# dedis/kyber

Hardware: AMD Instinct MI355X
Metric: scalar-muls/s + pairings/s per node; MSM sec at 2^20 points (higher is better)
Workload: dtype int32 limbs (radix 2^25.5), int64 accumulate; 1 GPU; Ed25519 batched fixed-base + var-base scalar-mul, 2^20 scalars per GPU (BASELINE.json configs[1]); elements_per_gpu=1048576

## Files before the change

kyber_amd/csrc/ed25519.hip:

```cpp
#ifndef KYB_TU_WAVES
#define KYB_TU_WAVES 2
#endif
#include "context.h"
#include "ed25519_dev.cuh"
#include "ed25519_launch.h"
#include "msm.cuh"
#include "ed25519_h2c.cuh"
#include <stdlib.h>
#include <string.h>

#include <algorithm>
#include <atomic>
#include <chrono>
#include <thread>
#include <vector>

namespace kyb {


template <int G = 2>
__global__ void ed25519_build_base_table_kernel(int32_t* __restrict__ tab, const uint32_t* __restrict__ point,
                                                uint32_t* __restrict__ ok, int rows = ED_TAB_POS * ED_TAB_ENT) {
    const int t = blockIdx.x * blockDim.x + threadIdx.x;
    if (t >= rows) return;
    ge_p3 B;
    if (point) {
        uint32_t pw[8];
        load_words8(pw, point);
        const bool good = ge_p3_fromwords(B, pw);
        if (t == 0) *ok = good ? 1u : 0u;
    } else {
        B.X = fe_bx(); B.Y = fe_by(); fe_1(B.Z); B.T = fe_bt();
    }
    ed_comb_row<G>(tab + (size_t)t * ED_TAB_STRIDE, t, B);
}

__global__ __launch_bounds__(64, KYB_TU_WAVES) void ed25519_encode_kernel(size_t n, const int32_t* __restrict__ proj,
                                                            const uint8_t* __restrict__ status,
                                                            uint32_t* __restrict__ out) {
    ed_encode_chunk(n, proj, (size_t)blockIdx.x * blockDim.x + threadIdx.x, [&](size_t i, uint32_t (&w)[8]) {
        if (status && status[i]) {
#pragma unroll
            for (int k = 0; k < 8; k++) w[k] = 0;
        }
        store_words8(out + i * 8, w);
    });
}


template <int G>
__global__ __launch_bounds__(256, 3) void ed25519_mul_base_kernel(
    size_t n, const uint32_t* __restrict__ scalars, uint32_t* __restrict__ out,
    const int32_t* __restrict__ tab, uint32_t flags, int32_t* __restrict__ proj) {
    const bool full = (flags & KYB_F_VARTIME) != 0;
    for (size_t idx = (size_t)blockIdx.x * blockDim.x + threadIdx.x; idx < n;
         idx += (size_t)gridDim.x * blockDim.x) {
        uint32_t a[8];
        load_words8(a, scalars + idx * 8);
        int8_t e[65];
        recode16(e, a, full);
        ge_p3 h;
        ge_p3_0(h);
        ge_precomp t;
        ge_p1p1 r;
        const int npos = full ? EdComb<G>::POS : EdComb<G>::POS_CT;
#pragma unroll 1
        for (int k = 0; k < npos; k++) {
            int d = 0;
#pragma unroll
            for (int i = G - 1; i >= 0; i--)
                if (G * k + i <= 64) d = 16 * d + (int)e[G * k + i];
            if (full && __ballot(d != 0) == 0) continue;
            select_precomp_tab<EdComb<G>::ENT>(t, tab, k, d);
            ge_madd(r, h, t);
            ge_p1p1_to_p3(h, r);
        }
        if (proj) {
            store_proj(proj, idx, h);
            continue;
        }
        uint32_t w[8];
        ge_p3_towords(w, h);
        store_words8(out + idx * 8, w);
    }
}

KYB_DEV void select_precomp_uniform(ge_precomp& t, const int32_t* __restrict__ tab, int i, int b) {
    const bool neg = b < 0;
    const int babs = neg ? -b : b;
    const int pos = i >> 1, mult = (i & 1) ? 16 : 1;
    fe_1(t.ypx);
    fe_1(t.ymx);
    fe_0(t.xy2d);
#pragma unroll 1
    for (int m = 1; m <= 8; m++) {
        const int4* e = reinterpret_cast<const int4*>(tab + (size_t)(pos * ED_TAB_ENT + (m * mult - 1)) * ED_TAB_STRIDE);
        int32_t w[32];
#pragma unroll
        for (int q = 0; q < 8; q++) {
            const int4 x = e[q];
            w[4 * q] = x.x;
            w[4 * q + 1] = x.y;
            w[4 * q + 2] = x.z;
            w[4 * q + 3] = x.w;
        }
        const int32_t keep = -(int32_t)(babs == m);
#pragma unroll
        for (int l = 0; l < 10; l++) {
            t.ypx.v[l] ^= (t.ypx.v[l] ^ w[l]) & keep;
            t.ymx.v[l] ^= (t.ymx.v[l] ^ w[10 + l]) & keep;
            t.xy2d.v[l] ^= (t.xy2d.v[l] ^ w[20 + l]) & keep;
        }
    }
    ge_precomp_cneg(t, neg);
}
__global__ __launch_bounds__(256, 3) void ed25519_mul_base_uniform_kernel(
    size_t n, const uint32_t* __restrict__ scalars, uint32_t* __restrict__ out,
    const int32_t* __restrict__ tab, int32_t* __restrict__ proj) {
    for (size_t idx = (size_t)blockIdx.x * blockDim.x + threadIdx.x; idx < n;
         idx += (size_t)gridDim.x * blockDim.x) {
        uint32_t a[8];
        load_words8(a, scalars + idx * 8);
        int8_t e[65];
        recode16(e, a, false);
        ge_p3 h;
        ge_p3_0(h);
        ge_precomp t;
        ge_p1p1 r;
#pragma unroll 1
        for (int i = 0; i < 64; i++) {
            select_precomp_uniform(t, tab, i, (int)e[i]);
            ge_madd(r, h, t);
            ge_p1p1_to_p3(h, r);
        }
        if (proj) {
            store_proj(proj, idx, h);
            continue;
        }
        uint32_t w[8];
        ge_p3_towords(w, h);
        store_words8(out + idx * 8, w);
    }
}


template <bool GTAB, bool UNI = false>
__global__ __launch_bounds__(128, 3) void ed25519_mul_kernel(
    size_t n, const uint32_t* __restrict__ scalars, const uint32_t* __restrict__ points,
    size_t points_stride, uint32_t* __restrict__ out, uint8_t* __restrict__ status,
    uint32_t flags, int32_t* __restrict__ proj, int4* __restrict__ gtab) {
    const size_t idx = (size_t)blockIdx.x * blockDim.x + threadIdx.x;
    if (idx >= n) return;
    const bool full = !UNI && (flags & KYB_F_VARTIME) != 0;
    uint32_t pw[8], a[8];
    load_words8(pw, points + idx * points_stride);
    load_words8(a, scalars + idx * 8);
    ge_p3 A;
    const bool ok = ge_p3_fromwords(A, pw);
    int8_t e[65];
    recode16(e, a, full);
    ge_p3 h;
    const int vt_top = full ? wave_top_digit(a) : 63;
    if constexpr (GTAB) {
        TabGlobal tab{gtab + idx * 80};
        ge_scalarmult_w4<UNI>(h, e, A, full, tab, vt_top);
    } else {
        TabScratch tab;
        ge_scalarmult_w4<UNI>(h, e, A, full, tab, vt_top);
    }
    if (proj) {
        store_proj(proj, idx, h);
        if (status) status[idx] = ok ? KYB_ST_OK : KYB_ST_BAD_POINT;
        return;
    }
    uint32_t w[8];
    ge_p3_towords(w, h);
    if (!ok) {
#pragma unroll
        for (int i = 0; i < 8; i++) w[i] = 0;
    }
    store_words8(out + idx * 8, w);
    if (status) status[idx] = ok ? KYB_ST_OK : KYB_ST_BAD_POINT;
}

int ed25519_build_tables(DeviceCtx* ctx) {
    KYB_HIP_CHECK(hipMalloc(&ctx->ed_base_tab, ED_TAB_WORDS * sizeof(int32_t)));
    hipLaunchKernelGGL(ed25519_build_base_table_kernel<2>, dim3((ED_TAB_POS * ED_TAB_ENT + 63) / 64), dim3(64), 0,
                       nullptr, ctx->ed_base_tab, (const uint32_t*)nullptr, (uint32_t*)nullptr, ED_TAB_POS * ED_TAB_ENT);
    KYB_HIP_CHECK(hipGetLastError());
    const auto t0 = std::chrono::steady_clock::now();
    KYB_HIP_CHECK(hipMalloc(&ctx->ed_wide_tab, ED_WIDE_WORDS * sizeof(int32_t)));
    hipLaunchKernelGGL(ed25519_build_base_table_kernel<ED_COMB_G>, dim3((EdWide::ROWS + 63) / 64), dim3(64), 0, nullptr,
                       ctx->ed_wide_tab, (const uint32_t*)nullptr, (uint32_t*)nullptr, EdWide::ROWS);
    KYB_HIP_CHECK(hipGetLastError());
    KYB_HIP_CHECK(hipStreamSynchronize(nullptr));
    ctx->ed_wide_build_us = std::chrono::duration_cast<std::chrono::microseconds>(std::chrono::steady_clock::now() - t0).count();
    return KYB_OK;
}
void ed25519_free_tables(DeviceCtx* ctx) {
    if (ctx->ed_base_tab) hipFree(ctx->ed_base_tab);
    if (ctx->ed_wide_tab) hipFree(ctx->ed_wide_tab);
    ctx->ed_base_tab = ctx->ed_wide_tab = nullptr;
}

constexpr size_t ENC_DEFER_MIN = 4096;


static int launch_mul_base(DeviceCtx* ctx, size_t n, const void* d_scalars, void* d_out, uint32_t flags,
                           hipStream_t st, const int32_t* tab = nullptr) {
    const bool wide = !tab && !(flags & KYB_F_UNIFORM);
    if (!tab) tab = wide ? ctx->ed_wide_tab : ctx->ed_base_tab;
    if (n == 0) return KYB_OK;
    const int block = 256;
    size_t want = (n + block - 1) / block;
    size_t cap = (size_t)ctx->num_cu * 8;
    int grid = (int)(want < cap ? want : cap);
    EdSlab w{};
    std::lock_guard<std::recursive_mutex> enq_lock(ctx->enq_mu);
    if (n >= ENC_DEFER_MIN)
        if (int rc = ed_slab(ctx, st, ED_SLAB_MUL_BASE, n, &w)) return rc;
    if (flags & KYB_F_UNIFORM) {
        hipLaunchKernelGGL(ed25519_mul_base_uniform_kernel, dim3(grid), dim3(block), 0, st, n,
                           (const uint32_t*)d_scalars, (uint32_t*)d_out, tab, w.proj);
    } else {
        const auto kernel = wide ? ed25519_mul_base_kernel<ED_COMB_G> : ed25519_mul_base_kernel<2>;
        hipLaunchKernelGGL(kernel, dim3(grid), dim3(block), 0, st, n, (const uint32_t*)d_scalars, (uint32_t*)d_out, tab,
                           flags, w.proj);
    }
    if (w.proj)
        hipLaunchKernelGGL(ed25519_encode_kernel, ed_encode_grid(n), dim3(ED_ENC_BLOCK), 0, st, n, w.proj,
                           (const uint8_t*)nullptr, (uint32_t*)d_out);
    KYB_HIP_CHECK(hipGetLastError());
    return KYB_OK;
}
static int launch_mul(size_t n, const void* d_scalars, const void* d_points, size_t stride, void* d_out,
                      void* d_status, uint32_t flags, hipStream_t st) {
    if (n == 0) return KYB_OK;
    const int block = 128;
    size_t grid = (n + block - 1) / block;
    EdSlab w{};
    uint8_t* stat = (uint8_t*)d_status;
    DeviceCtx* ctx;
    int rc = get_ctx(&ctx);
    if (rc) return rc;
    std::lock_guard<std::recursive_mutex> enq_lock(ctx->enq_mu);
    const bool defer = n >= ENC_DEFER_MIN, uni = (flags & KYB_F_UNIFORM) != 0;
    const auto kernel = defer ? (uni ? ed25519_mul_kernel<true, true> : ed25519_mul_kernel<true, false>)
                              : (uni ? ed25519_mul_kernel<false, true> : ed25519_mul_kernel<false, false>);
    if (defer) {
        if ((rc = ed_slab(ctx, st, ed_slab_mul(stat == nullptr), n, &w))) return rc;
        if (!stat) stat = w.status;
    }
    hipLaunchKernelGGL(kernel, dim3((unsigned)grid), dim3(block), 0, st, n, (const uint32_t*)d_scalars,
                       (const uint32_t*)d_points, stride, (uint32_t*)d_out, stat, flags, w.proj, w.gtab);
    if (w.proj)
        hipLaunchKernelGGL(ed25519_encode_kernel, ed_encode_grid(n), dim3(ED_ENC_BLOCK), 0, st, n, w.proj,
                           (const uint8_t*)stat, (uint32_t*)d_out);
    KYB_HIP_CHECK(hipGetLastError());
    return KYB_OK;
}

}

using namespace kyb;

static bool ed_mul_flags_bad(uint32_t flags) {
    return (flags & ~(KYB_F_VARTIME | KYB_F_UNIFORM)) || (flags & (KYB_F_VARTIME | KYB_F_UNIFORM)) == (KYB_F_VARTIME | KYB_F_UNIFORM);
}

extern "C" {

int kyb_ed25519_mul_base_dev(size_t n, const void* d_scalars, void* d_out, uint32_t flags, void* stream) {
    if ((n && (!d_scalars || !d_out)) || ed_mul_flags_bad(flags)) {
        set_error("kyb_ed25519_mul_base_dev: bad argument");
        return KYB_E_ARG;
    }
    DeviceCtx* ctx;
    int rc = get_ctx(&ctx);
    if (rc) return rc;
    return launch_mul_base(ctx, n, d_scalars, d_out, flags, (hipStream_t)stream);
}

int kyb_ed25519_mul_dev(size_t n, const void* d_scalars, const void* d_points, void* d_out, void* d_status,
                        uint32_t flags, void* stream) {
    if ((n && (!d_scalars || !d_points || !d_out)) || ed_mul_flags_bad(flags)) {
        set_error("kyb_ed25519_mul_dev: bad argument");
        return KYB_E_ARG;
    }
    DeviceCtx* ctx;
    int rc = get_ctx(&ctx);
    if (rc) return rc;
    return launch_mul(n, d_scalars, d_points, 8, d_out, d_status, flags, (hipStream_t)stream);
}

static int mul_host(size_t n, const uint8_t* scalars, const uint8_t* points, size_t stride, uint8_t* out,
                    uint8_t* status, uint32_t flags);

int kyb_ed25519_mul_base(size_t n, const uint8_t* scalars, uint8_t* out, uint32_t flags) {
    if ((n && (!scalars || !out)) || ed_mul_flags_bad(flags)) {
        set_error("kyb_ed25519_mul_base: bad argument");
        return KYB_E_ARG;
    }
    if (n == 0) return KYB_OK;
    if (md_active(n))
        return md_run(n, [&](int, size_t lo, size_t hi) { return kyb_ed25519_mul_base(hi - lo, scalars + 32 * lo, out + 32 * lo, flags); });
    return mul_host(n, scalars, nullptr, 0, out, nullptr, flags);
}

constexpr size_t PIPE_CHUNK_MAX = PIN_SLOT_ELEMS;
constexpr int PIPE_SLOTS = DeviceCtx::NPIN, PIPE_STREAMS = 3;
static size_t pipe_chunk(const DeviceCtx* ctx) {
    if (const char* e = getenv("KYB_PIPE_CHUNK")) {
        const size_t v = (size_t)strtoull(e, nullptr, 10) & ~size_t(63);
        if (v >= 4096) return std::min(PIPE_CHUNK_MAX, v);
    }
    (void)ctx;
    return size_t(1) << 17;
}
static int pipe_nstreams() {
    if (const char* e = getenv("KYB_PIPE_STREAMS")) {
        const int v = atoi(e);
        if (v >= 1 && v <= PIPE_STREAMS) return v;
    }
    return 2;
}
constexpr size_t SAME_BASE_TABLE_MIN = 16384;

static int pipe_streams(DeviceCtx::StagePool* pool) {
    for (int i = 0; i < PIPE_STREAMS; i++)
        if (!pool->pipe[i]) KYB_HIP_CHECK(hipStreamCreateWithFlags(&pool->pipe[i], hipStreamNonBlocking));
    return KYB_OK;
}

static int mul_host(size_t n, const uint8_t* scalars, const uint8_t* points, size_t stride, uint8_t* out,
                    uint8_t* status, uint32_t flags) {
    DeviceCtx* ctx;
    int rc = get_ctx(&ctx);
    if (rc) return rc;
    bool fixed = points == nullptr;
    const size_t npts = fixed ? 0 : (stride ? n : 1);
    StageScope sc_(ctx);
    StageBuf d_s, d_p, d_o, d_st, d_tab;
    if ((rc = d_s.alloc(n * 32))) return rc;
    if ((rc = d_p.alloc(npts * 32))) return rc;
    if ((rc = d_o.alloc(n * 32))) return rc;
    if ((rc = d_st.alloc(n))) return rc;
    const int32_t* tab = nullptr;
    if (!fixed && !stride && (n >= SAME_BASE_TABLE_MIN || (flags & KYB_F_UNIFORM))) {
        if ((rc = d_tab.alloc(ED_TAB_WORDS * sizeof(int32_t) + 256))) return rc;
        uint32_t* d_ok = (uint32_t*)((uint8_t*)d_tab.p + ED_TAB_WORDS * sizeof(int32_t));
        KYB_HIP_CHECK(hipMemcpy(d_p.p, points, 32, hipMemcpyHostToDevice));
        hipLaunchKernelGGL(ed25519_build_base_table_kernel<2>, dim3((ED_TAB_POS * ED_TAB_ENT + 63) / 64), dim3(64), 0, sc_.stream(),
                           (int32_t*)d_tab.p, (const uint32_t*)d_p.p, d_ok, ED_TAB_POS * ED_TAB_ENT);
        uint32_t ok = 0;
        KYB_HIP_CHECK(hipMemcpy(&ok, d_ok, 4, hipMemcpyDeviceToHost));
        if (!ok) {
            memset(out, 0, n * 32);
            if (status) memset(status, KYB_ST_BAD_POINT, n);
            return KYB_OK;
        }
        if (status) memset(status, 0, n);
        tab = (const int32_t*)d_tab.p;
        fixed = true;
    }
    auto launch = [&](size_t off, size_t cnt, hipStream_t st) -> int {
        uint8_t* s = (uint8_t*)d_s.p + off * 32;
        uint8_t* o = (uint8_t*)d_o.p + off * 32;
        if (fixed) return launch_mul_base(ctx, cnt, s, o, flags, st, tab);
        const uint8_t* p = (const uint8_t*)d_p.p + (stride ? off * 32 : 0);
        return launch_mul(cnt, s, p, stride, o, (uint8_t*)d_st.p + off, flags, st);
    };
    const size_t PIPE_CHUNK = pipe_chunk(ctx);
    if (n < 2 * PIPE_CHUNK) {
        KYB_HIP_CHECK(hipMemcpy(d_s.p, scalars, n * 32, hipMemcpyHostToDevice));
        if (npts) KYB_HIP_CHECK(hipMemcpy(d_p.p, points, npts * 32, hipMemcpyHostToDevice));
        if ((rc = launch(0, n, nullptr))) return rc;
        if ((rc = d_o.download(out, n * 32))) return rc;
        if (status && !fixed) rc = d_st.download(status, n);
        return rc;
    }
    DeviceCtx::StagePool* pool = sc_.pool;
    if ((rc = pipe_streams(pool))) return rc;
    const int nstreams = pipe_nstreams();
    const bool per_point = !fixed && stride;
    const bool want_status = status && !fixed;
    if ((rc = ctx_pin_slots(pool))) return rc;
    const size_t nchunks = (n + PIPE_CHUNK - 1) / PIPE_CHUNK;
    std::vector<hipEvent_t> ev_out(nchunks);
    for (size_t i = 0; i < nchunks; i++) KYB_HIP_CHECK(hipEventCreateWithFlags(&ev_out[i], hipEventDisableTiming));
    auto enqueue = [&](size_t i) -> int {
        const size_t off = i * PIPE_CHUNK, cnt = std::min(PIPE_CHUNK, n - off);
        uint8_t* pin = (uint8_t*)pool->pin_in[i % PIPE_SLOTS];
        uint8_t* pout = (uint8_t*)pool->pin_out[i % PIPE_SLOTS];
        hipStream_t s_k = pool->pipe[i % nstreams];
        par_memcpy(pin, scalars + off * 32, cnt * 32);
        if (per_point) par_memcpy(pin + PIPE_CHUNK_MAX * 32, points + off * 32, cnt * 32);
        int r;
        if (fixed) {
            r = launch_mul_base(ctx, cnt, pin, pout, flags, s_k, tab);
        } else {
            const uint8_t* p = per_point ? pin + PIPE_CHUNK_MAX * 32 : (const uint8_t*)d_p.p;
            r = launch_mul(cnt, pin, p, stride, pout, (uint8_t*)d_st.p + off, flags, s_k);
        }
        if (r) return r;
        if (want_status)
            KYB_HIP_CHECK(hipMemcpyAsync(pout + PIPE_CHUNK_MAX * 32, (uint8_t*)d_st.p + off, cnt, hipMemcpyDeviceToHost, s_k));
        KYB_HIP_CHECK(hipEventRecord(ev_out[i], s_k));
        return KYB_OK;
    };
    auto drain = [&](size_t i) -> int {
        const size_t off = i * PIPE_CHUNK, cnt = std::min(PIPE_CHUNK, n - off);
        KYB_HIP_CHECK(hipEventSynchronize(ev_out[i]));
        const uint8_t* pout = (const uint8_t*)pool->pin_out[i % PIPE_SLOTS];
        par_memcpy(out + off * 32, pout, cnt * 32);
        if (want_status) memcpy(status + off, pout + PIPE_CHUNK_MAX * 32, cnt);
        return KYB_OK;
    };
    if (!fixed && !stride) KYB_HIP_CHECK(hipMemcpy(d_p.p, points, 32, hipMemcpyHostToDevice));
    std::atomic<size_t> enqueued{0}, drained{0};
    std::atomic<int> drain_rc{KYB_OK};
    std::atomic<bool> stop{false};
    const int device = ctx->device;
    std::string drain_err;
    std::thread drainer([&] {
        if (hipSetDevice(device) != hipSuccess) {
            drain_err = "ed25519 host pipeline: hipSetDevice failed on the drain thread";
            drain_rc.store(KYB_E_HIP);
            return;
        }
        for (size_t i = 0; i < nchunks; i++) {
            while (enqueued.load(std::memory_order_acquire) <= i) {
                if (stop.load(std::memory_order_acquire)) return;
                std::this_thread::yield();
            }
            const int r = drain(i);
            if (r) {
                drain_err = kyb_last_error();
                drain_rc.store(r);
                return;
            }
            drained.store(i + 1, std::memory_order_release);
        }
    });
    for (size_t i = 0; i < nchunks && rc == KYB_OK; i++) {
        while (i >= (size_t)PIPE_SLOTS && drained.load(std::memory_order_acquire) + PIPE_SLOTS <= i && drain_rc.load() == KYB_OK)
            std::this_thread::yield();
        if (drain_rc.load() != KYB_OK) break;
        rc = enqueue(i);
        if (rc == KYB_OK) enqueued.store(i + 1, std::memory_order_release);
    }
    if (rc != KYB_OK) stop.store(true, std::memory_order_release);
    drainer.join();
    if (rc == KYB_OK && (rc = drain_rc.load()) != KYB_OK) set_error(drain_err);
    hipError_t e2 = hipSuccess;
    for (int i = 0; i < PIPE_STREAMS; i++) {
        const hipError_t e = hipStreamSynchronize(pool->pipe[i]);
        if (e != hipSuccess) e2 = e;
    }
    for (size_t i = 0; i < nchunks; i++) hipEventDestroy(ev_out[i]);
    if (rc == KYB_OK && e2 != hipSuccess) {
        set_error("ed25519 host pipeline: stream synchronisation failed");
        rc = KYB_E_HIP;
    }
    return rc;
}

int kyb_ed25519_mul(size_t n, const uint8_t* scalars, const uint8_t* points, uint8_t* out, uint8_t* status,
                    uint32_t flags) {
    if ((n && (!scalars || !points || !out)) || ed_mul_flags_bad(flags)) {
        set_error("kyb_ed25519_mul: bad argument");
        return KYB_E_ARG;
    }
    if (n == 0) return KYB_OK;
    if (md_active(n))
        return md_run(n, [&](int, size_t lo, size_t hi) {
            return kyb_ed25519_mul(hi - lo, scalars + 32 * lo, points + 32 * lo, out + 32 * lo, status ? status + lo : nullptr, flags);
        });
    return mul_host(n, scalars, points, 8, out, status, flags);
}

int kyb_ed25519_mul_same_base(size_t n, const uint8_t* scalars, const uint8_t point[32], uint8_t* out,
                              uint8_t* status, uint32_t flags) {
    if ((n && (!scalars || !out)) || !point || ed_mul_flags_bad(flags)) {
        set_error("kyb_ed25519_mul_same_base: bad argument");
        return KYB_E_ARG;
    }
    if (n == 0) return KYB_OK;
    if (md_active(n))
        return md_run(n, [&](int, size_t lo, size_t hi) {
            return kyb_ed25519_mul_same_base(hi - lo, scalars + 32 * lo, point, out + 32 * lo, status ? status + lo : nullptr, flags);
        });
    return mul_host(n, scalars, point, 0, out, status, flags);
}

int kyb_ed25519_debug_base_table(int32_t* out) {
    if (!out) return KYB_E_ARG;
    DeviceCtx* ctx;
    int rc = get_ctx(&ctx);
    if (rc) return rc;
    KYB_HIP_CHECK(hipMemcpy(out, ctx->ed_base_tab, ED_TAB_WORDS * sizeof(int32_t), hipMemcpyDeviceToHost));
    return KYB_OK;
}

int kyb_ed25519_comb_info(int64_t info[6]) {
    if (!info) return KYB_E_ARG;
    DeviceCtx* ctx;
    int rc = get_ctx(&ctx);
    if (rc) return rc;
    info[0] = ED_COMB_G;
    info[1] = EdWide::POS;
    info[2] = EdWide::ENT;
    info[3] = EdWide::LAST_ENT;
    info[4] = (int64_t)(ED_WIDE_WORDS * sizeof(int32_t));
    info[5] = ctx->ed_wide_build_us;
    return KYB_OK;
}

int kyb_ed25519_debug_comb_table(int pos, int row0, int nrows, int32_t* out) {
    if (!out || pos < 0 || pos >= EdWide::POS || row0 < 0 || nrows < 0 ||
        row0 + nrows > (pos == EdWide::POS - 1 ? EdWide::LAST_ENT : EdWide::ENT)) {
        set_error("kyb_ed25519_debug_comb_table: bad argument");
        return KYB_E_ARG;
    }
    DeviceCtx* ctx;
    int rc = get_ctx(&ctx);
    if (rc) return rc;
    const size_t off = ((size_t)pos * EdWide::ENT + row0) * ED_TAB_STRIDE;
    KYB_HIP_CHECK(hipMemcpy(out, ctx->ed_wide_tab + off, (size_t)nrows * ED_TAB_STRIDE * sizeof(int32_t), hipMemcpyDeviceToHost));
    return KYB_OK;
}
}

namespace kyb {
struct EdMsm {
    using Aff = ge_precomp;
    using Acc = ge_p3;
    static constexpr int WIRE = 32, OUT = 32;
    static constexpr bool SCALAR_BE = false;
    static constexpr uint32_t COMBINE_FLAGS = 0;
    static constexpr int DECODE_WAVES = 3;
    __host__ __device__ static size_t wire_size(uint32_t) { return 32; }
    __device__ static int decode(Aff& a, const uint8_t* wire, uint32_t) {
        uint32_t w[8];
        load_words8(w, reinterpret_cast<const uint32_t*>(wire));
        ge_p3 p;
        const bool ok = ge_p3_fromwords(p, w);
        fe one;
        fe_1(one);
        fe_add(a.ypx, p.Y, p.X);
        fe_sub(a.ymx, p.Y, p.X);
        fe_mul(a.ypx, a.ypx, one);
        fe_mul(a.ymx, a.ymx, one);
        fe_mul(a.xy2d, p.T, fe_d2());
        return ok ? KYB_ST_OK : KYB_ST_BAD_POINT;
    }
    __device__ static void scalar_words(uint32_t (&k)[8], const uint8_t* wire) {
        load_words8(k, reinterpret_cast<const uint32_t*>(wire));
    }
    static constexpr bool HAS_EFFECTIVE = true;
    __device__ static void effective(uint32_t (&k)[8], Aff& p, int bits) {
        if (bits < 253) return;
        if (ed_effective_scalar(k)) ge_precomp_cneg(p, true);
    }
    __device__ static void identity(Acc& a) { ge_p3_0(a); }
    __device__ static void madd(Acc& acc, const Aff& p, bool neg) {
        ge_precomp t = p;
        ge_precomp_cneg(t, neg);
        ge_p1p1 r;
        ge_madd(r, acc, t);
        ge_p1p1_to_p3(acc, r);
    }
    __device__ static void add(Acc& r, const Acc& a, const Acc& b) {
        ge_cached c;
        ge_p3_to_cached(c, b);
        ge_p1p1 t;
        ge_add(t, a, c);
        ge_p1p1_to_p3(r, t);
    }
    __device__ static void dbl(Acc& r, const Acc& a) {
        ge_p1p1 t;
        ge_dbl(t, a.X, a.Y, a.Z);
        ge_p1p1_to_p3(r, t);
    }
    static constexpr int COOP = 4;
    using Field = fe;
    __device__ static void dbl_coop(Acc& s, int r, fe* sh) {
        fe in = s.X, t, m;
        fe_add(t, s.X, s.Y);
        fe_cmov(in, s.Y, r == 1);
        fe_cmov(in, s.Z, r == 2);
        fe_cmov(in, t, r == 3);
        fe_sq_sel(m, in, r == 2);
        sh[r] = m;
        __syncthreads();
        const fe XX = sh[0], YY = sh[1], ZZ2 = sh[2], t0 = sh[3];
        __syncthreads();
        fe Xp, Yp, Zp, Tp;
        fe_add(Yp, YY, XX);
        fe_sub(Zp, YY, XX);
        fe_sub(Xp, t0, Yp);
        fe_sub(Tp, ZZ2, Zp);
        fe a = Xp, b = Tp;
        fe_cmov(a, Yp, r == 1);
        fe_cmov(a, Zp, r == 2);
        fe_cmov(b, Zp, r == 1);
        fe_cmov(b, Yp, r == 3);
        fe_mul(m, a, b);
        sh[r] = m;
        __syncthreads();
        s.X = sh[0];
        s.Y = sh[1];
        s.Z = sh[2];
        s.T = sh[3];
        __syncthreads();
    }
    __device__ static void encode(uint8_t* out, const Acc& a) {
        uint32_t w[8];
        ge_p3_towords(w, a);
        store_words8(reinterpret_cast<uint32_t*>(out), w);
    }
};
}

extern "C" {
int kyb_ed25519_msm(size_t n, const uint8_t* scalars, const uint8_t* points, uint8_t out[32], uint8_t* status) {
    return kyb::msm::run_host<kyb::EdMsm>(n, scalars, points, out, status);
}
int kyb_ed25519_msm_flags(size_t n, const uint8_t* scalars, const uint8_t* points, uint8_t out[32], uint8_t* status,
                          uint32_t flags) {
    if (flags & ~KYB_F_SCALAR_BITS_MASK) {
        kyb::set_error("kyb_ed25519_msm_flags: only KYB_F_SCALAR_BITS applies");
        return KYB_E_ARG;
    }
    return kyb::msm::run_host<kyb::EdMsm>(n, scalars, points, out, status, flags);
}
int kyb_ed25519_poly_eval(size_t n, const uint32_t* idx, size_t t, const uint8_t* commits, uint8_t* out, uint8_t* status) {
    return kyb::msm::poly_eval_host<kyb::EdMsm>(n, idx, t, commits, out, status, 0);
}
int kyb_ed25519_poly_eval_dev(size_t n, const void* d_idx, size_t t, const void* d_commits, void* d_out, void* d_status,
                              void* stream) {
    kyb::DeviceCtx* ctx;
    int rc = kyb::get_ctx(&ctx);
    if (rc) return rc;
    return kyb::msm::poly_eval_run<kyb::EdMsm>(ctx, n, d_idx, t, d_commits, d_out, d_status, 0, (hipStream_t)stream);
}
int kyb_ed25519_msm_dev(size_t n, const void* d_scalars, const void* d_points, void* d_out, void* d_status,
                        void* stream) {
    kyb::DeviceCtx* ctx;
    int rc = kyb::get_ctx(&ctx);
    if (rc) return rc;
    return kyb::msm::run<kyb::EdMsm>(ctx, n, d_scalars, d_points, d_out, d_status, (hipStream_t)stream);
}
}

namespace kyb {
__global__ __launch_bounds__(64, KYB_TU_WAVES) void ed25519_hash_kernel(size_t n, const uint8_t* __restrict__ msgs, size_t msg_len,
                                                          EdDstArg dst, uint8_t* __restrict__ out) {
    const size_t idx = (size_t)blockIdx.x * blockDim.x + threadIdx.x;
    if (idx >= n) return;
    ed_hash_wire(out + 32 * idx, msgs + msg_len * idx, msg_len, dst);
}
}

extern "C" {
int kyb_ed25519_hash_dev(size_t n, const void* d_msgs, size_t msg_len, const uint8_t* dst, size_t dst_len, void* d_out,
                         void* stream) {
    if ((n && ((!d_msgs && msg_len) || !d_out)) || !dst || dst_len == 0 || dst_len > 255) {
        kyb::set_error("kyb_ed25519_hash_dev: bad argument (the domain separation tag must be 1..255 bytes)");
        return KYB_E_ARG;
    }
    if (!n) return KYB_OK;
    kyb::EdDstArg d;
    memset(&d, 0, sizeof d);
    memcpy(d.b, dst, dst_len);
    d.len = (uint32_t)dst_len;
    hipLaunchKernelGGL(kyb::ed25519_hash_kernel, dim3((unsigned)((n + 63) / 64)), dim3(64), 0, (hipStream_t)stream, n,
                       (const uint8_t*)d_msgs, msg_len, d, (uint8_t*)d_out);
    KYB_HIP_CHECK(hipGetLastError());
    return KYB_OK;
}
int kyb_ed25519_hash(size_t n, const uint8_t* msgs, size_t msg_len, const uint8_t* dst, size_t dst_len, uint8_t* out) {
    if (n && ((!msgs && msg_len) || !out)) {
        kyb::set_error("kyb_ed25519_hash: bad argument");
        return KYB_E_ARG;
    }
    if (!n) return KYB_OK;
    kyb::DeviceCtx* ctx;
    int rc = kyb::get_ctx(&ctx);
    if (rc) return rc;
    return kyb::staged_call(ctx, {{msgs, n * msg_len}}, {{out, n * 32}}, [&](void* const* in, void* const* o, hipStream_t st) {
        return kyb_ed25519_hash_dev(n, in[0], msg_len, dst, dst_len, o[0], st);
    });
}
}

namespace kyb {
__global__ __launch_bounds__(128, KYB_TU_WAVES) void ed25519_add_kernel(size_t n, const uint32_t* __restrict__ a,
                                                          const uint32_t* __restrict__ b, uint32_t* __restrict__ out,
                                                          uint8_t* __restrict__ status) {
    const size_t idx = (size_t)blockIdx.x * blockDim.x + threadIdx.x;
    if (idx >= n) return;
    uint32_t wa[8], wb[8], w[8];
    load_words8(wa, a + idx * 8);
    load_words8(wb, b + idx * 8);
    ge_p3 A, B, R;
    const bool ok = ge_p3_fromwords(A, wa) & ge_p3_fromwords(B, wb);
    ge_cached c;
    ge_p3_to_cached(c, B);
    ge_p1p1 t;
    ge_add(t, A, c);
    ge_p1p1_to_p3(R, t);
    ge_p3_towords(w, R);
    if (!ok) {
#pragma unroll
        for (int i = 0; i < 8; i++) w[i] = 0;
    }
    store_words8(out + idx * 8, w);
    if (status) status[idx] = ok ? KYB_ST_OK : KYB_ST_BAD_POINT;
}
__global__ __launch_bounds__(128, KYB_TU_WAVES) void ed25519_unmarshal_kernel(size_t n, const uint32_t* __restrict__ in,
                                                                uint32_t* __restrict__ out,
                                                                uint8_t* __restrict__ status) {
    const size_t idx = (size_t)blockIdx.x * blockDim.x + threadIdx.x;
    if (idx >= n) return;
    uint32_t w[8];
    load_words8(w, in + idx * 8);
    ge_p3 A;
    const bool ok = ge_p3_fromwords(A, w);
    ge_p3_towords(w, A);
    if (!ok) {
#pragma unroll
        for (int i = 0; i < 8; i++) w[i] = 0;
    }
    store_words8(out + idx * 8, w);
    if (status) status[idx] = ok ? KYB_ST_OK : KYB_ST_BAD_POINT;
}
}
extern "C" {
int kyb_ed25519_unmarshal_dev(size_t n, const void* d_points, void* d_out, void* d_status, void* stream) {
    if (n && (!d_points || !d_out)) {
        kyb::set_error("kyb_ed25519_unmarshal_dev: bad argument");
        return KYB_E_ARG;
    }
    if (!n) return KYB_OK;
    hipLaunchKernelGGL(kyb::ed25519_unmarshal_kernel, dim3((unsigned)((n + 127) / 128)), dim3(128), 0,
                       (hipStream_t)stream, n, (const uint32_t*)d_points, (uint32_t*)d_out, (uint8_t*)d_status);
    KYB_HIP_CHECK(hipGetLastError());
    return KYB_OK;
}
int kyb_ed25519_unmarshal(size_t n, const uint8_t* points, uint8_t* out, uint8_t* status) {
    if (n && (!points || !out)) {
        kyb::set_error("kyb_ed25519_unmarshal: bad argument");
        return KYB_E_ARG;
    }
    if (!n) return KYB_OK;
    kyb::DeviceCtx* ctx;
    int rc = kyb::get_ctx(&ctx);
    if (rc) return rc;
    return kyb::staged_call(ctx, {{points, n * 32}}, {{out, n * 32}, {status, n}}, [&](void* const* in, void* const* o, hipStream_t st) {
        return kyb_ed25519_unmarshal_dev(n, in[0], o[0], o[1], st);
    });
}
int kyb_ed25519_add_dev(size_t n, const void* d_a, const void* d_b, void* d_out, void* d_status, void* stream) {
    if (n && (!d_a || !d_b || !d_out)) {
        kyb::set_error("kyb_ed25519_add_dev: bad argument");
        return KYB_E_ARG;
    }
    if (!n) return KYB_OK;
    hipLaunchKernelGGL(kyb::ed25519_add_kernel, dim3((unsigned)((n + 127) / 128)), dim3(128), 0, (hipStream_t)stream, n,
                       (const uint32_t*)d_a, (const uint32_t*)d_b, (uint32_t*)d_out, (uint8_t*)d_status);
    KYB_HIP_CHECK(hipGetLastError());
    return KYB_OK;
}
int kyb_ed25519_add(size_t n, const uint8_t* a, const uint8_t* b, uint8_t* out, uint8_t* status) {
    if (n && (!a || !b || !out)) {
        kyb::set_error("kyb_ed25519_add: bad argument");
        return KYB_E_ARG;
    }
    if (!n) return KYB_OK;
    kyb::DeviceCtx* ctx;
    int rc = kyb::get_ctx(&ctx);
    if (rc) return rc;
    return kyb::staged_call(ctx, {{a, n * 32}, {b, n * 32}}, {{out, n * 32}, {status, n}}, [&](void* const* in, void* const* o, hipStream_t st) {
        return kyb_ed25519_add_dev(n, in[0], in[1], o[0], o[1], st);
    });
}
}
```

kyber_amd/csrc/ed25519_dev.cuh:

```cuda
#pragma once
#include "ge25519.cuh"

#if !defined(__HIPCC__)
#include <type_traits>
struct int4 { int32_t x, y, z, w; };
struct uint4 { uint32_t x, y, z, w; };
inline int4 make_int4(int32_t x, int32_t y, int32_t z, int32_t w) { return int4{x, y, z, w}; }
inline uint4 make_uint4(uint32_t x, uint32_t y, uint32_t z, uint32_t w) { return uint4{x, y, z, w}; }
#define KYB_DEV_CONST static
#else
#define KYB_DEV_CONST __device__
#endif

namespace kyb {

constexpr int ED_TAB_POS = 33;
constexpr int ED_TAB_ENT = 136;
constexpr int ED_TAB_STRIDE = 32;
constexpr int ED_TAB_WORDS = ED_TAB_POS * ED_TAB_ENT * ED_TAB_STRIDE;

template <int G>
struct EdComb {
    static constexpr int POS = (65 + G - 1) / G;
    static constexpr int POS_CT = (64 + G - 1) / G;
    static constexpr int ENT = 8 * ((1 << (4 * G)) - 1) / 15;
    static constexpr int LAST_D = 65 - G * (POS - 1);
    static constexpr int LAST_ENT = 8 * ((1 << (4 * LAST_D)) - 1) / 15;
    static constexpr int ROWS = (POS - 1) * ENT + LAST_ENT;
};
#ifndef ED_COMB_G
#define ED_COMB_G 4
#endif
using EdWide = EdComb<ED_COMB_G>;
constexpr size_t ED_WIDE_WORDS = (size_t)EdWide::ROWS * ED_TAB_STRIDE;

KYB_DEV void load_words8(uint32_t w[8], const uint32_t* __restrict__ p) {
    const uint4 a = reinterpret_cast<const uint4*>(p)[0];
    const uint4 b = reinterpret_cast<const uint4*>(p)[1];
    w[0] = a.x; w[1] = a.y; w[2] = a.z; w[3] = a.w;
    w[4] = b.x; w[5] = b.y; w[6] = b.z; w[7] = b.w;
}
KYB_DEV void store_words8(uint32_t* __restrict__ p, const uint32_t w[8]) {
    reinterpret_cast<uint4*>(p)[0] = make_uint4(w[0], w[1], w[2], w[3]);
    reinterpret_cast<uint4*>(p)[1] = make_uint4(w[4], w[5], w[6], w[7]);
}

template <int G>
KYB_DEV void ed_comb_row(int32_t* __restrict__ o, int t, const ge_p3& B) {
    constexpr int ENT = EdComb<G>::ENT;
    const int pos = t / ENT, j = t - pos * ENT;
    ge_cached cB;
    ge_p3_to_cached(cB, B);
    ge_p3 acc;
    ge_p3_0(acc);
    ge_p1p1 r;
#pragma unroll 1
    for (int bit = 4 * G - 1; bit >= 0; bit--) {
        ge_dbl(r, acc.X, acc.Y, acc.Z);
        ge_p1p1_to_p3(acc, r);
        if (((j + 1) >> bit) & 1) {
            ge_add(r, acc, cB);
            ge_p1p1_to_p3(acc, r);
        }
    }
#pragma unroll 1
    for (int k = 0; k < 4 * G * pos; k++) {
        ge_dbl(r, acc.X, acc.Y, acc.Z);
        ge_p1p1_to_p3(acc, r);
    }
    fe zi, x, y, ypx, ymx, xy2d, z;
    fe_invert(zi, acc.Z);
    fe_mul(x, acc.X, zi);
    fe_mul(y, acc.Y, zi);
    fe_add(ypx, y, x);
    fe_sub(ymx, y, x);
    fe_mul(xy2d, x, y);
    fe_mul(xy2d, xy2d, fe_d2());
    fe_1(z);
    fe_mul(ypx, ypx, z);
    fe_mul(ymx, ymx, z);
#pragma unroll
    for (int l = 0; l < 10; l++) {
        o[l] = ypx.v[l];
        o[10 + l] = ymx.v[l];
        o[20 + l] = xy2d.v[l];
    }
    o[30] = o[31] = 0;
}

constexpr int ENC_CHUNK = 16;

KYB_DEV void store_proj(int32_t* __restrict__ proj, size_t idx, const ge_p3& h) {
    int32_t* o = proj + idx * 30;
#pragma unroll
    for (int l = 0; l < 10; l++) {
        o[l] = h.X.v[l];
        o[10 + l] = h.Y.v[l];
        o[20 + l] = h.Z.v[l];
    }
}
KYB_DEV void load_fe(fe& f, const int32_t* __restrict__ p) {
#pragma unroll
    for (int l = 0; l < 10; l++) f.v[l] = p[l];
}
template <class Emit>
KYB_DEV void ed_encode_chunk(size_t n, const int32_t* __restrict__ proj, size_t lane, Emit emit) {
    const size_t lo = lane * ENC_CHUNK;
    if (lo >= n) return;
    const int cnt = (int)((n - lo) < (size_t)ENC_CHUNK ? (n - lo) : (size_t)ENC_CHUNK);
    fe pre[ENC_CHUNK];
    fe z, acc;
    load_fe(acc, proj + lo * 30 + 20);
    pre[0] = acc;
#pragma unroll 1
    for (int j = 1; j < cnt; j++) {
        load_fe(z, proj + (lo + j) * 30 + 20);
        fe_mul(acc, acc, z);
        pre[j] = acc;
    }
    fe inv;
    fe_invert(inv, acc);
#pragma unroll 1
    for (int j = cnt - 1; j >= 0; j--) {
        fe zi, X, Y;
        load_fe(z, proj + (lo + j) * 30 + 20);
        if (j > 0) {
            fe_mul(zi, inv, pre[j - 1]);
            fe_mul(inv, inv, z);
        } else {
            zi = inv;
        }
        load_fe(X, proj + (lo + j) * 30);
        load_fe(Y, proj + (lo + j) * 30 + 10);
        uint32_t w[8];
        ge_encode_with_zinv(w, X, Y, zi);
        emit(lo + j, w);
    }
}

template <int ENT>
KYB_DEV void select_precomp_tab(ge_precomp& t, const int32_t* __restrict__ tab, int pos, int b) {
    const bool neg = b < 0;
    const int babs = neg ? -b : b;
    const int4* e = reinterpret_cast<const int4*>(tab + (size_t)(pos * ENT + (babs ? babs - 1 : 0)) * ED_TAB_STRIDE);
    int32_t w[32];
#pragma unroll
    for (int i = 0; i < 8; i++) {
        const int4 x = e[i];
        w[4 * i] = x.x;
        w[4 * i + 1] = x.y;
        w[4 * i + 2] = x.z;
        w[4 * i + 3] = x.w;
    }
#pragma unroll
    for (int l = 0; l < 10; l++) {
        t.ypx.v[l] = w[l];
        t.ymx.v[l] = w[10 + l];
        t.xy2d.v[l] = w[20 + l];
    }
    if (babs == 0) {
        fe_1(t.ypx);
        fe_1(t.ymx);
        fe_0(t.xy2d);
    }
    ge_precomp_cneg(t, neg);
}

struct TabScratch {
    ge_cached tab[8];
    KYB_DEV void put(int j, const ge_cached& c) { tab[j] = c; }
    KYB_DEV void get(ge_cached& c, int j) const { c = tab[j]; }
};
struct TabGlobal {
    int4* base;
    KYB_DEV void put(int j, const ge_cached& c) {
        int4* q = base + j * 10;
        const fe* f[4] = {&c.YpX, &c.YmX, &c.Z, &c.T2d};
        int32_t w[40];
#pragma unroll
        for (int k = 0; k < 4; k++)
#pragma unroll
            for (int l = 0; l < 10; l++) w[10 * k + l] = f[k]->v[l];
#pragma unroll
        for (int i = 0; i < 10; i++) q[i] = make_int4(w[4 * i], w[4 * i + 1], w[4 * i + 2], w[4 * i + 3]);
    }
    KYB_DEV void get(ge_cached& c, int j) const {
        const int4* q = base + j * 10;
        int32_t w[40];
#pragma unroll
        for (int i = 0; i < 10; i++) {
            const int4 x = q[i];
            w[4 * i] = x.x;
            w[4 * i + 1] = x.y;
            w[4 * i + 2] = x.z;
            w[4 * i + 3] = x.w;
        }
        fe* f[4] = {&c.YpX, &c.YmX, &c.Z, &c.T2d};
#pragma unroll
        for (int k = 0; k < 4; k++)
#pragma unroll
            for (int l = 0; l < 10; l++) f[k]->v[l] = w[10 * k + l];
    }
    KYB_DEV void get_signed(ge_cached& c, int b) const;
};
KYB_DEV_CONST __attribute__((aligned(16))) const int32_t ED_CACHED_IDENTITY[40] = {1, 0, 0, 0, 0, 0, 0, 0, 0, 0,
                                                                               1, 0, 0, 0, 0, 0, 0, 0, 0, 0,
                                                                               1};
KYB_DEV void TabGlobal::get_signed(ge_cached& c, int b) const {
    const bool neg = b < 0;
    const int babs = neg ? -b : b;
#if defined(__HIPCC__)
    typedef int32_t i32x2 __attribute__((ext_vector_type(2)));
    typedef int32_t i32x4 __attribute__((ext_vector_type(4)));
    using gint = const __attribute__((address_space(1))) int32_t;
    using gint2 = const __attribute__((address_space(1))) i32x2;
    using gint4 = const __attribute__((address_space(1))) i32x4;
#else
    struct i32x2 { int32_t x, y; };
    struct i32x4 { int32_t x, y, z, w; };
    using gint = const int32_t;
    using gint2 = const i32x2;
    using gint4 = const i32x4;
#endif
    gint* e = babs ? (gint*)(base + (babs - 1) * 10) : (gint*)ED_CACHED_IDENTITY;
    gint2* p = (gint2*)(e + (neg ? 10 : 0));
    gint2* m = (gint2*)(e + (neg ? 0 : 10));
    gint4* q = (gint4*)(e + 20);
#pragma unroll
    for (int i = 0; i < 5; i++) {
        const i32x2 x = p[i], y = m[i];
        c.YpX.v[2 * i] = x.x;
        c.YpX.v[2 * i + 1] = x.y;
        c.YmX.v[2 * i] = y.x;
        c.YmX.v[2 * i + 1] = y.y;
    }
    int32_t w[20];
#pragma unroll
    for (int i = 0; i < 5; i++) {
        const i32x4 x = q[i];
        w[4 * i] = x.x;
        w[4 * i + 1] = x.y;
        w[4 * i + 2] = x.z;
        w[4 * i + 3] = x.w;
    }
    const int32_t s = -(int32_t)neg;
#pragma unroll
    for (int l = 0; l < 10; l++) {
        c.Z.v[l] = w[l];
        c.T2d.v[l] = (w[10 + l] ^ s) - s;
    }
}
template <bool UNI = false, class Tab>
KYB_DEV void select_cached(ge_cached& c, const Tab& tab, int b) {
    const bool neg = b < 0;
    const int babs = neg ? -b : b;
    if constexpr (UNI) {
        ge_cached_0(c);
#pragma unroll 1
        for (int m = 1; m <= 8; m++) {
            ge_cached x;
            tab.get(x, m - 1);
            const int32_t keep = -(int32_t)(babs == m);
#pragma unroll
            for (int l = 0; l < 10; l++) {
                c.YpX.v[l] ^= (c.YpX.v[l] ^ x.YpX.v[l]) & keep;
                c.YmX.v[l] ^= (c.YmX.v[l] ^ x.YmX.v[l]) & keep;
                c.Z.v[l] ^= (c.Z.v[l] ^ x.Z.v[l]) & keep;
                c.T2d.v[l] ^= (c.T2d.v[l] ^ x.T2d.v[l]) & keep;
            }
        }
    } else if constexpr (std::is_same_v<Tab, TabGlobal>) {
        tab.get_signed(c, b);
        return;
    } else {
        tab.get(c, babs ? babs - 1 : 0);
        if (babs == 0) ge_cached_0(c);
    }
    ge_cached_cneg(c, neg);
}

KYB_DEV int wave_top_digit(const uint32_t a[8]) {
    int bits = 0;
#pragma unroll
    for (int i = 0; i < 8; i++)
        if (a[i]) bits = 32 * i + 32 - __builtin_clz(a[i]);
    int t = (bits + 3) >> 2;
    if (t > 64) t = 64;
#if defined(__HIP_DEVICE_COMPILE__)
#pragma unroll
    for (int off = 32; off >= 1; off >>= 1) {
        const int o = __shfl_xor(t, off, 64);
        t = o > t ? o : t;
    }
    t = __builtin_amdgcn_readfirstlane(t);
#endif
    return t;
}

template <class Tab>
KYB_DEV void ge_window_table(Tab& tab, const ge_p3& A) {
    ge_p1p1 t;
    ge_p3 u;
    ge_cached c;
    ge_p3_to_cached(c, A);
    tab.put(0, c);
#pragma unroll 1
    for (int i = 0; i < 7; i++) {
        ge_add(t, A, c);
        ge_p1p1_to_p3(u, t);
        ge_p3_to_cached(c, u);
        tab.put(i + 1, c);
    }
}

template <bool UNI = false, class Tab>
KYB_DEV void ge_scalarmult_w4(ge_p3& h, const int8_t e[65], const ge_p3& A, bool full, Tab& tab, int vt_top) {
    ge_p1p1 t;
    ge_p3 u;
    ge_p2 r;
    ge_cached c;
    ge_window_table(tab, A);
    ge_p3_0(u);
    int top = 63;
    if (full) top = vt_top;
    select_cached<UNI>(c, tab, e[top]);
    ge_add(t, u, c);
    uint32_t pk[8];
#pragma unroll
    for (int j = 0; j < 8; j++) {
        pk[j] = 0;
#pragma unroll
        for (int q = 0; q < 8; q++) pk[j] |= (uint32_t)((e[8 * j + q] + 8) & 15) << (4 * q);
    }
    auto shl4 = [&pk]() {
#pragma unroll
        for (int j = 7; j > 0; j--) pk[j] = (pk[j] << 4) | (pk[j - 1] >> 28);
        pk[0] <<= 4;
    };
#pragma unroll 1
    for (int i = top; i < 64; i++) shl4();
#pragma unroll 1
    for (int i = top - 1; i >= 0; i--) {
        const int d = (int)(pk[7] >> 28) - 8;
        shl4();
        ge_p1p1_to_p2(r, t);
        ge_dbl(t, r.X, r.Y, r.Z);
        ge_p1p1_to_p2(r, t);
        ge_dbl(t, r.X, r.Y, r.Z);
        ge_p1p1_to_p2(r, t);
        ge_dbl(t, r.X, r.Y, r.Z);
        ge_p1p1_to_p2(r, t);
        ge_dbl(t, r.X, r.Y, r.Z);
#if defined(__HIP_DEVICE_COMPILE__)
        if (!UNI && full && __ballot(d != 0) == 0) continue;
#endif
        ge_p1p1_to_p3(u, t);
        select_cached<UNI>(c, tab, d);
        ge_add(t, u, c);
    }
    ge_p1p1_to_p3(h, t);
}

}
```

Baseline: 169.2 million scalar-muls/s.

## Pack comb digits into registers and build window table with mixed additions

Replaces per-iteration dynamic indexing of the int8 digit array in the fixed-base comb kernels with a packed 32-bit register shifter, so the digit array no longer has to sit in scratch memory. The variable-base window table is now built with mixed addition (ge_madd against the affine base, Z=1 after decoding) instead of full projective addition, which saves field multiplications per table entry. This assumes the decoded point has Z=1, and the packed digit path adds shift work and a tail special case on every iteration.

```diff
diff --git a/kyber_amd/csrc/ed25519.hip b/kyber_amd/csrc/ed25519.hip
--- a/kyber_amd/csrc/ed25519.hip
+++ b/kyber_amd/csrc/ed25519.hip
@@ -64,12 +64,10 @@
         ge_precomp t;
         ge_p1p1 r;
         const int npos = full ? EdComb<G>::POS : EdComb<G>::POS_CT;
+        EdCombDigits<G> digits(e);
 #pragma unroll 1
         for (int k = 0; k < npos; k++) {
-            int d = 0;
-#pragma unroll
-            for (int i = G - 1; i >= 0; i--)
-                if (G * k + i <= 64) d = 16 * d + (int)e[G * k + i];
+            const int d = digits.next(k);
             if (full && __ballot(d != 0) == 0) continue;
             select_precomp_tab<EdComb<G>::ENT>(t, tab, k, d);
             ge_madd(r, h, t);
@@ -127,9 +125,10 @@
         ge_p3_0(h);
         ge_precomp t;
         ge_p1p1 r;
+        EdCombDigits<1> digits(e);
 #pragma unroll 1
         for (int i = 0; i < 64; i++) {
-            select_precomp_uniform(t, tab, i, (int)e[i]);
+            select_precomp_uniform(t, tab, i, digits.next(i));
             ge_madd(r, h, t);
             ge_p1p1_to_p3(h, r);
         }
@@ -163,10 +162,10 @@
     const int vt_top = full ? wave_top_digit(a) : 63;
     if constexpr (GTAB) {
         TabGlobal tab{gtab + idx * 80};
-        ge_scalarmult_w4<UNI>(h, e, A, full, tab, vt_top);
+        ge_scalarmult_w4<UNI, true>(h, e, A, full, tab, vt_top);
     } else {
         TabScratch tab;
-        ge_scalarmult_w4<UNI>(h, e, A, full, tab, vt_top);
+        ge_scalarmult_w4<UNI, true>(h, e, A, full, tab, vt_top);
     }
     if (proj) {
         store_proj(proj, idx, h);
diff --git a/kyber_amd/csrc/ed25519_dev.cuh b/kyber_amd/csrc/ed25519_dev.cuh
--- a/kyber_amd/csrc/ed25519_dev.cuh
+++ b/kyber_amd/csrc/ed25519_dev.cuh
@@ -165,6 +165,45 @@
     }
     ge_precomp_cneg(t, neg);
 }
+
+KYB_DEV void ed_pack_digits(uint32_t pk[8], const int8_t e[65]) {
+#pragma unroll
+    for (int j = 0; j < 8; j++) {
+        pk[j] = 0;
+#pragma unroll
+        for (int q = 0; q < 8; q++) pk[j] |= (uint32_t)((e[8 * j + q] + 8) & 15) << (4 * q);
+    }
+}
+
+template <int G>
+struct EdCombDigits {
+    static_assert(G >= 1 && G <= 7, "a position's digits are read from one 32-bit word");
+    static constexpr int PACKED = 63 / G;
+    static constexpr int TAIL = EdComb<G>::POS - PACKED;
+    uint32_t pk[8];
+    int tail[TAIL];
+    KYB_DEV explicit EdCombDigits(const int8_t e[65]) {
+        ed_pack_digits(pk, e);
+#pragma unroll
+        for (int t = 0; t < TAIL; t++) {
+            int d = 0;
+#pragma unroll
+            for (int i = G - 1; i >= 0; i--)
+                if (G * (PACKED + t) + i <= 64) d = 16 * d + (int)e[G * (PACKED + t) + i];
+            tail[t] = d;
+        }
+    }
+    KYB_DEV int next(int k) {
+        int d = (int)(pk[0] & ((1u << (4 * G)) - 1u)) - EdComb<G>::ENT;
+#pragma unroll
+        for (int j = 0; j < 7; j++) pk[j] = (pk[j] >> (4 * G)) | (pk[j + 1] << (32 - 4 * G));
+        pk[7] >>= 4 * G;
+#pragma unroll
+        for (int t = 0; t < TAIL; t++)
+            if (k == PACKED + t) d = tail[t];
+        return d;
+    }
+};
 
 struct TabScratch {
     ge_cached tab[8];
@@ -297,41 +336,48 @@
     return t;
 }
 
-template <class Tab>
+template <bool AFFINE = false, class Tab>
 KYB_DEV void ge_window_table(Tab& tab, const ge_p3& A) {
     ge_p1p1 t;
     ge_p3 u;
     ge_cached c;
     ge_p3_to_cached(c, A);
     tab.put(0, c);
-#pragma unroll 1
-    for (int i = 0; i < 7; i++) {
-        ge_add(t, A, c);
-        ge_p1p1_to_p3(u, t);
-        ge_p3_to_cached(c, u);
-        tab.put(i + 1, c);
-    }
-}
-
-template <bool UNI = false, class Tab>
+    if constexpr (AFFINE) {
+        const ge_precomp a{c.YpX, c.YmX, c.T2d};
+        u = A;
+#pragma unroll 1
+        for (int i = 0; i < 7; i++) {
+            ge_madd(t, u, a);
+            ge_p1p1_to_p3(u, t);
+            ge_p3_to_cached(c, u);
+            tab.put(i + 1, c);
+        }
+    } else {
+#pragma unroll 1
+        for (int i = 0; i < 7; i++) {
+            ge_add(t, A, c);
+            ge_p1p1_to_p3(u, t);
+            ge_p3_to_cached(c, u);
+            tab.put(i + 1, c);
+        }
+    }
+}
+
+template <bool UNI = false, bool AFFINE = false, class Tab>
 KYB_DEV void ge_scalarmult_w4(ge_p3& h, const int8_t e[65], const ge_p3& A, bool full, Tab& tab, int vt_top) {
     ge_p1p1 t;
     ge_p3 u;
     ge_p2 r;
     ge_cached c;
-    ge_window_table(tab, A);
+    ge_window_table<AFFINE>(tab, A);
     ge_p3_0(u);
     int top = 63;
     if (full) top = vt_top;
     select_cached<UNI>(c, tab, e[top]);
     ge_add(t, u, c);
     uint32_t pk[8];
-#pragma unroll
-    for (int j = 0; j < 8; j++) {
-        pk[j] = 0;
-#pragma unroll
-        for (int q = 0; q < 8; q++) pk[j] |= (uint32_t)((e[8 * j + q] + 8) & 15) << (4 * q);
-    }
+    ed_pack_digits(pk, e);
     auto shl4 = [&pk]() {
 #pragma unroll
         for (int j = 7; j > 0; j--) pk[j] = (pk[j] << 4) | (pk[j - 1] >> 28);
```

Measured after the change: 172.0 million scalar-muls/s, median of 6. +1.7%, better.
